# marcottelab/FluorosequencingImageAnalysis

Measured on AMD Instinct MI355X. Metric: psf_lm_fits_per_sec, higher is better.
Workload: dtype f64

## Files before the change

### fluorosequencingimageanalysis_amd/csrc/fsq_fit_rounds.hip

```cpp
#include <algorithm>
#include <atomic>
#include <cstdlib>

#include <mutex>
#include <new>
#include <vector>

#include "fsq_common.h"
#include "fsq_lm_quad.h"

namespace {

#define WAVE_SYNC() do { __builtin_amdgcn_fence(__ATOMIC_RELEASE, "wavefront"); __builtin_amdgcn_wave_barrier(); \
                         __builtin_amdgcn_fence(__ATOMIC_ACQUIRE, "wavefront"); } while (0)

#ifdef FSQ_DEBUG_HZ
__device__ unsigned long long g_hz[32];
#endif
#ifdef FSQ_PHASE_PROFILE
__device__ unsigned long long g_rphase[32];
#define RPH_DECL unsigned long long rph_t0 = clock64(), rph_acc[16] = {0,0,0,0,0,0,0,0,0,0,0,0,0,0,0,0};
#define RPH_MARK(k) { unsigned long long t_ = clock64(); rph_acc[k] += t_ - rph_t0; rph_t0 = t_; }
#define RPH_FLUSH(off) if (threadIdx.x == 0 && (blockIdx.x & 63) == 0) { for (int k_ = 0; k_ < 16; k_++) atomicAdd(&g_rphase[(off) + k_], rph_acc[k_]); }
#else
#define RPH_DECL
#define RPH_MARK(k)
#define RPH_FLUSH(off)
#endif

enum { CNT_A = 0, CNT_BLO = 1, CNT_BHI = 2, CNT_C1 = 3, CNT_C3 = 4, CNT_SET = 8 };
enum { Q_EPS = Q_WA3 };
enum { A_IDX = 0, A_X = 1, A_DIAG = 8, A_LLIM1 = 15, A_FNORM = 16, A_PAR = 17, A_DELTA = 18, A_XNORM = 19, A_ITER = 20,
       A_HDR = 21 , A_E = 21 , A_LEN = 46,
       B_GNORM = 21, B_IPVT = 22, B_QTF = 23, B_SDIAG = 30, B_R = 37, B_LEN = 65,
       C_PARL = 65, C_PARU = 66, C_FP = 67, C_LMIT = 68, C_LEN = 69 };

struct FitOut {
    double x[FSQ_NP];
    int status, niter, nfev, pad;
};
struct FitStat {
    double vmax, vmean;
};

struct Ctx {
    uint16_t* roi;
    int pix32;
    FitOut* out;
    FitStat* stat;
    long long cap;
    long long pool;
    int* err;
    int* slow_total;
    int* done;
    int tshift;
    int wave_prio;
    int force_redo;
    int force_slow_mod;
};

enum { G_KINIT_POS = 1, G_KINIT_SLOT = 2, G_KA_BLO = 3, G_KA_BHI = 4, G_KA_OVERLAP = 5, G_KA_SLOW = 6, G_KB_C1 = 7, G_KB_C3 = 8, G_KB_A = 9,
       G_KB_BLO = 10, G_KB_BHI = 11 };
FSQ_DEV long long fsq_guard(const Ctx& c, long long v, long long limit, int code)
{
    if ((unsigned long long)v < (unsigned long long)limit) return v;
    atomicMax(c.err, code);
    return 0;
}

FSQ_DEV int wave_reserve(int* counter, bool want)
{
    const unsigned long long m = __ballot(want);
    if (m == 0) return 0;
    const int lane = threadIdx.x & 63;
    const int leader = __ffsll((long long)m) - 1;
    int base = 0;
    if (lane == leader) base = atomicAdd(counter, __popcll(m));
    base = __shfl(base, leader);
    return base + __popcll(m & ((1ull << lane) - 1ull));
}

FSQ_DEV long long wave_reserve_checked(const Ctx& c, int* counter, bool want, long long limit, int code)
{
    const int at = wave_reserve(counter, want);
    return want ? fsq_guard(c, at, limit, code) : 0;
}

struct BatchArgs {
    const uint16_t* src; const int32_t* cand; int H, W; long long n; int from_image;
    int pix_fmt;
    long long base;
    int ticket;
    int no_queue;
};

FSQ_DEV void wave_mark_done(int* done, bool term, int ticket)
{
    unsigned long long m = __ballot(term);
    const int lane = threadIdx.x & 63;
    while (m) {
        const int leader = __ffsll((long long)m) - 1;
        const int t = __shfl(ticket, leader);
        const unsigned long long mm = __ballot(term && ticket == t);
        if (lane == leader) atomicAdd(done + t, __popcll(mm));
        m &= ~mm;
    }
}

#ifndef FSQ_NT
#define FSQ_NT 0
#endif
typedef unsigned fsq_u4v __attribute__((ext_vector_type(4)));
FSQ_DEV double nt_ld(const double* p) { return FSQ_NT ? __builtin_nontemporal_load(p) : *p; }
FSQ_DEV void nt_st(double* p, double v) { if (FSQ_NT) __builtin_nontemporal_store(v, p); else *p = v; }
FSQ_DEV uint4 nt_ld4(const void* p)
{
    const fsq_u4v v = FSQ_NT ? __builtin_nontemporal_load((const fsq_u4v*)p) : *(const fsq_u4v*)p;
    return make_uint4(v.x, v.y, v.z, v.w);
}
FSQ_DEV void nt_st4(void* p, uint4 w)
{
    fsq_u4v v; v.x = w.x; v.y = w.y; v.z = w.z; v.w = w.w;
    if (FSQ_NT) __builtin_nontemporal_store(v, (fsq_u4v*)p); else *(fsq_u4v*)p = v;
}
struct NtRef {
    double* p;
    FSQ_DEV operator double() const { return nt_ld(p); }
    FSQ_DEV void operator=(double v) const { nt_st(p, v); }
};
struct NtQ {
    double* p;
    FSQ_DEV NtRef operator[](long long i) const { return NtRef{p + i}; }
};
FSQ_DEV NtQ ntq(const double* p) { return NtQ{const_cast<double*>(p)}; }

FSQ_DEV int tag_slot(const Ctx& c, int tag) { return (int)((unsigned)tag & ((1u << c.tshift) - 1u)); }
FSQ_DEV int tag_ticket(const Ctx& c, int tag) { return (int)((unsigned)tag >> c.tshift); }

FSQ_DEV int rpk(int i, int k) { return i * 7 - (i * (i - 1)) / 2 + (k - i); }
FSQ_DEV double pack2(int a, int b) { return __longlong_as_double(((long long)(unsigned)a) | ((long long)b << 32)); }
FSQ_DEV void unpack2(double v, int* a, int* b) { long long u = __double_as_longlong(v); *a = (int)(unsigned)(u & 0xffffffffll); *b = (int)(u >> 32); }

FSQ_DEV void roi_pixels(const BatchArgs& c, long long idx, double* d)
{
    if (c.from_image) {
        const int f = c.cand[3 * idx], h = c.cand[3 * idx + 1], w = c.cand[3 * idx + 2];
        const size_t base = ((size_t)f * c.H + (h - 2)) * c.W + (w - 2);
#pragma unroll
        for (int a = 0; a < 5; a++)
#pragma unroll
            for (int b = 0; b < 5; b++) d[a * 5 + b] = (double)fsq_pixel(c.src, base + (size_t)a * c.W + b, c.pix_fmt);
    } else {
#pragma unroll
        for (int k = 0; k < FSQ_NPIX; k++) d[k] = (double)c.src[idx * FSQ_NPIX + k];
    }
}

FSQ_DEV void roi_compact(const Ctx& c, long long idx, double* d)
{
    if (c.pix32) {
        const uint32_t* s32 = (const uint32_t*)c.roi + (size_t)idx * 32;
#pragma unroll
        for (int k = 0; k < FSQ_NPIX; k++) d[k] = (double)s32[k];
        return;
    }
    const uint16_t* src = c.roi + (size_t)idx * 32;
    const uint4 a = nt_ld4(src), b = nt_ld4(src + 8), e = nt_ld4(src + 16), f = nt_ld4(src + 24);
    const unsigned w[16] = {a.x, a.y, a.z, a.w, b.x, b.y, b.z, b.w, e.x, e.y, e.z, e.w, f.x, f.y, f.z, f.w};
#pragma unroll
    for (int k = 0; k < FSQ_NPIX; k++) d[k] = (double)((w[k >> 1] >> (16 * (k & 1))) & 0xffffu);
}

__global__ void __launch_bounds__(256) kinit(Ctx c, BatchArgs b, double* __restrict__ QA, int* __restrict__ cntA)
{
    const long long i0 = (long long)blockIdx.x * blockDim.x + threadIdx.x;
    const bool ok = i0 < b.n;
    const long long i = ok ? i0 : 0;
    const long long pos = wave_reserve_checked(c, cntA, ok && !b.no_queue, c.cap, G_KINIT_POS);
    if (b.n <= 0) return;
    const long long slot = fsq_guard(c, b.base + i, c.pool, G_KINIT_SLOT);
    double v[FSQ_NPIX];
    roi_pixels(b, i, v);
    if (ok && c.pix32) {
        uint32_t* dst = (uint32_t*)c.roi + (size_t)slot * 32;
#pragma unroll
        for (int k = 0; k < 32; k++) dst[k] = (k < FSQ_NPIX) ? (unsigned)v[k] : 0u;
    } else if (ok) {
        unsigned w[16];
#pragma unroll
        for (int k = 0; k < 16; k++) {
            unsigned lo = (2 * k < FSQ_NPIX) ? (unsigned)v[2 * k] : 0u, hi = (2 * k + 1 < FSQ_NPIX) ? (unsigned)v[2 * k + 1] : 0u;
            w[k] = lo | (hi << 16);
        }
        uint16_t* dst = c.roi + (size_t)slot * 32;
        nt_st4(dst, make_uint4(w[0], w[1], w[2], w[3])); nt_st4(dst + 8, make_uint4(w[4], w[5], w[6], w[7]));
        nt_st4(dst + 16, make_uint4(w[8], w[9], w[10], w[11])); nt_st4(dst + 24, make_uint4(w[12], w[13], w[14], w[15]));
    }
    double mx = v[0], isum = 0.0;
#pragma unroll
    for (int k = 0; k < FSQ_NPIX; k++) { mx = v[k] > mx ? v[k] : mx; isum += v[k]; }
#pragma unroll
    for (int pass = 0; pass < FSQ_NPIX; pass++)
#pragma unroll
        for (int k = (pass & 1); k + 1 < FSQ_NPIX; k += 2) {
// ... 62 lines not shown
}
template <int G>
FSQ_DEV double kag_dot25(const double* lds, int grp, int off)
{
    double S[4];
#pragma unroll
    for (int l = 0; l < 4; l++) {
        double a = QL(off, l), b = QL(off, 4 + l), c = QL(off, 8 + l), e = QL(off, 12 + l);
        S[l] = ((a * a + b * b) + c * c) + e * e;
    }
    double d = (S[0] + S[2]) + (S[1] + S[3]);
#pragma unroll
    for (int i = 16; i < 25; i++) { double v = QL(off, i); d = fsq_fma(v, v, d); }
    return d;
}

#define KA_ROWS(i) do { if (L == 8 && ((i) % 5) == 4) __builtin_amdgcn_sched_barrier(0); } while (0)
#define KA_PIN(v) do { if (FAST) asm volatile("" : "+v"(v)); } while (0)
#ifdef FSQ_DEBUG_HZ
#define KA_HZ(code, cond) do { if (cond) { hz = true; if (FAST) atomicAdd(&g_hz[code], 1ull); } } while (0)
#else
#define KA_HZ(code, cond) do { if (cond) hz = true; } while (0)
#endif
template <bool FAST, int L, bool P32 = false>
__global__ void __launch_bounds__(64, (L == 8 ? 4 : 2)) kA_jacobian(Ctx c, const double* __restrict__ QA, const int* __restrict__ cntA_p,
                                                                    double* __restrict__ QB, int* __restrict__ cnt_cur,
                                                                    double* __restrict__ SQ, int* __restrict__ slow_cnt,
                                                                    int* __restrict__ next_counters)
{
    constexpr int G = 64 / L;
    constexpr int NC = 8 / L;
    constexpr int MPX = (FSQ_NPIX + L - 1) / L;
    constexpr int MREC = (A_HDR + L - 1) / L;
    __shared__ double lds[Q_KA_END * G];
    const int lane = threadIdx.x, grp = lane / L, cl = lane % L, gbase = lane - cl;
    const int n7 = FSQ_NP;
    if (c.wave_prio) __builtin_amdgcn_s_setprio(3);
    const int cntA = FAST ? *cntA_p : *slow_cnt;
    if (!FAST && blockIdx.x == 0 && threadIdx.x == 0 && cntA > 0) atomicAdd(c.slow_total, cntA);
    if (FAST && blockIdx.x == 0 && threadIdx.x < CNT_SET) next_counters[threadIdx.x] = 0;
    double col[NC][FSQ_NPIX];
    RPH_DECL
    const long long cap = c.cap;
    const int stride = gridDim.x * G;
    int base = blockIdx.x * G;
    if (base >= cntA) return;
    do {
        RPH_MARK(0)
        const bool active = (base + grp) < cntA;
        const NtQ qa = ntq(QA + (active ? base + grp : 0));
        double rec[MREC];
#pragma unroll
        for (int m = 0; m < MREC; m++) { const int f = cl + L * m; rec[m] = (active && f < A_HDR) ? (double)qa[f * cap] : 0.0; }
        bool hz = false, qhz = false;
        int emin = 0;
        int tag, niter, nfev, hist;
        unpack2(__shfl(rec[A_IDX / L], gbase + A_IDX % L), &tag, &hist);
        unpack2(__shfl(rec[A_ITER / L], gbase + A_ITER % L), &niter, &nfev);
        const bool b_hi = hist > 1;
        const int at_lo = wave_reserve(cnt_cur + CNT_BLO, active && cl == 0 && !b_hi);
        const int at_hi = wave_reserve(cnt_cur + CNT_BHI, active && cl == 0 && b_hi);
#ifdef FSQ_EXPERIMENT_EXTRA_ATOMICS_KA
        {
            int sink = 0;
            for (int x = 0; x < FSQ_EXPERIMENT_EXTRA_ATOMICS_KA; x++) sink += wave_reserve(cnt_cur + 5 + (x & 1), active && cl == 0);
            if (sink == 0x7fffffff) atomicMax(c.err, 99);
        }
#endif
        if (active && cl == 0) {
            if (!b_hi) fsq_guard(c, at_lo, cap, G_KA_BLO); else fsq_guard(c, at_hi, cap, G_KA_BHI);
            if ((long long)at_lo + (long long)at_hi + 2 > cap && (at_lo > 0 || at_hi > 0)) {
                const int nlo = b_hi ? cnt_cur[CNT_BLO] : at_lo + 1, nhi = b_hi ? at_hi + 1 : cnt_cur[CNT_BHI];
                if ((long long)nlo + nhi > cap) atomicMax(c.err, (int)G_KA_OVERLAP);
            }
        }
        const long long at = __shfl((active && cl == 0) ? (int)fsq_guard(c, b_hi ? (long long)(cap - 1) - at_hi : (long long)at_lo, cap, b_hi ? G_KA_BHI : G_KA_BLO) : 0, gbase);
        const int idx = tag_slot(c, tag);
        const bool fresh = active && (nfev == 0);
        double llim1 = 0., fnorm = 0., xnorm = 0., delta = 0., par_in = 0.;
        unsigned ipvt = 0x76543210u;
        int status = 0;
        double gnorm = 0.;
        uint4 roi = make_uint4(0u, 0u, 0u, 0u);
        uint4 roi_hi = make_uint4(0u, 0u, 0u, 0u);
        double ev[MPX];
#pragma unroll
        for (int m = 0; m < MPX; m++) ev[m] = 0.0;
        if (active) {
            if (P32) {
                static_assert(!P32 || L == 4, "32-bit pixels: the four-lane Jacobian round only");
                const uint32_t* r32 = (const uint32_t*)c.roi + (size_t)idx * 32 + cl * 8;
                roi = nt_ld4(r32); roi_hi = nt_ld4(r32 + 4);
            } else if (L == 4) roi = nt_ld4(c.roi + (size_t)idx * 32 + cl * 8);
            else {
                const unsigned long long w8 = fsq_bits(nt_ld((const double*)(c.roi + (size_t)idx * 32 + cl * 4)));
                roi.x = (unsigned)w8; roi.y = (unsigned)(w8 >> 32);
            }
            if (!fresh) {
#pragma unroll
                for (int m = 0; m < MPX; m++) { const int k = cl + L * m; if (k < FSQ_NPIX) ev[m] = qa[(A_E + k) * cap]; }
            }
#pragma unroll
            for (int m = 0; m < MREC; m++) {
                const int f = cl + L * m;
                if (f >= 1 && f <= 19) QL(Q_X, f - 1) = rec[m];
            }
        }
        WAVE_SYNC();
        RPH_MARK(1)
        if (active) {
            double xx[FSQ_NP], hh[FSQ_NP];
#pragma unroll
            for (int k = 0; k < FSQ_NP; k++) {
                xx[k] = QL(Q_X, k);
                const double eps = 1.4901161193847656e-08;
                double h_ = eps * __builtin_fabs(xx[k]);
                if (h_ == 0) h_ = eps;
                const double ul = k < 2 ? 0.0 : k < 4 ? 3.0 : k < 6 ? 2.0 : 360.0;
                if (k >= 2 && (xx[k] > ul - h_)) h_ = -h_;
                hh[k] = h_;
            }
            bool bad = false;
            double sn, cs;
            fsq_sincos(FSQ_PI_180 * xx[6], &sn, &cs);
            const double rcx = xx[3] * cs - xx[2] * sn, rcy = xx[3] * sn + xx[2] * cs;
            const FsqDivisor k4 = fsq_divisor(xx[4]), k5 = fsq_divisor(xx[5]);
            if (FAST)
                hz = hz || !fsq_divisor_in_range(xx[4]) || !fsq_divisor_in_range(xx[5]) || !(__builtin_fabs(xx[2]) <= 0x1p100) ||
                     !(__builtin_fabs(xx[3]) <= 0x1p100);
            {
                const unsigned w[4] = {roi.x, roi.y, roi.z, roi.w};
                const unsigned w32[8] = {roi.x, roi.y, roi.z, roi.w, roi_hi.x, roi_hi.y, roi_hi.z, roi_hi.w};
#pragma unroll
                for (int t = 0; t < 32 / L; t++) {
                    const int k = cl * (32 / L) + t;
                    if (k < FSQ_NPIX) QL(Q_DATA, k) = P32 ? (double)w32[t & 7] : (double)((w[t >> 1] >> (16 * (t & 1))) & 0xffffu);
                }
                if (!fresh) {
#pragma unroll
                    for (int m = 0; m < MPX; m++) { const int k = cl + L * m; if (k < FSQ_NPIX) QL(Q_FVEC, k) = ev[m]; }
                }
            }
            WAVE_SYNC();
            if (__ballot(fresh)) {
                if (fresh) {
#pragma unroll 1
                    for (int m = 0; m < MPX; m++) {
                        const int i = cl + L * m;
                        if (i < FSQ_NPIX) {
                            const int xi = i / 5;
                            const double x = (double)xi, y = (double)(i - 5 * xi);
                            const double xp = x * cs - y * sn, yp = x * sn + y * cs;
                            const double E = ka_gauss<FAST>(rcx - xp, rcy - yp, k4, k5, &emin, &bad);
                            QL(Q_FVEC, i) = E;
                        }
                    }
                }
                WAVE_SYNC();
            }
            if (fresh) nfev = 1;
            {
                const double x2p = xx[2] + hh[2], x3p = xx[3] + hh[3];
                const double rcx2 = xx[3] * cs - x2p * sn, rcy2 = xx[3] * sn + x2p * cs;
                const double rcx3 = x3p * cs - xx[2] * sn, rcy3 = x3p * sn + xx[2] * cs;
                if (FAST) KA_HZ(0, !(__builtin_fabs(x2p) <= 0x1p100) || !(__builtin_fabs(x3p) <= 0x1p100));
#pragma unroll 1
                for (int m = 0; m < MPX; m++) {
                    const int i = cl + L * m;
                    if (i < FSQ_NPIX) {
                        const int xi = i / 5;
                        const double x = (double)xi, y = (double)(i - 5 * xi);
                        const double xp = x * cs - y * sn, yp = x * sn + y * cs;
                        const double d = QL(Q_DATA, i);
                        const double E2 = ka_gauss<FAST>(rcx2 - xp, rcy2 - yp, k4, k5, &emin, &bad);
                        const double E3 = ka_gauss<FAST>(rcx3 - xp, rcy3 - yp, k4, k5, &emin, &bad);
                        QL(Q_STAGE, i) = d - (xx[0] + xx[1] * E2);
                        QL(Q_STAGE + 25, i) = d - (xx[0] + xx[1] * E3);
                    }
                }
                const double p0 = (cl == 0) ? xx[0] + hh[0] : xx[0], p1 = (cl == 1) ? xx[1] + hh[1] : xx[1];
#pragma unroll
                for (int i = 0; i < FSQ_NPIX; i++) { col[0][i] = QL(Q_DATA, i) - (p0 + p1 * QL(Q_FVEC, i)); KA_ROWS(i); }
                WAVE_SYNC();
// ... 342 lines not shown
                    col[pass][FSQ_NPIX - 1] = 0.0;
                }
                WAVE_SYNC();
                RPH_MARK(11)
            }
            RPH_MARK(4)
#define QRG(i, k) QL(Q_R, (i) * 7 + nib_get(ipvt, (k)))
            llim1 = QL(Q_TMP, 0); fnorm = QL(Q_TMP, 1); par_in = QL(Q_TMP, 2); delta = QL(Q_TMP, 3); xnorm = QL(Q_TMP, 4);
            if (niter == 1) {
#pragma unroll
                for (int k = 0; k < FSQ_NP; k++) {
                    double a = QL(Q_ACN, k);
                    double dg = (a == 0) ? 1. : a;
                    QL(Q_DIAG, k) = dg;
                    QL(Q_WA3, k) = dg * QL(Q_X, k);
                }
                xnorm = fsq_sqrt(kag_dot7<G>(lds, grp, Q_WA3));
                delta = 100. * xnorm;
                if (delta == 0.) delta = 100.;
            }
            gnorm = 0.;
            if (fnorm != 0) {
                for (int j = 0; j < n7; j++) {
                    double an = QL(Q_ACN, nib_get(ipvt, j));
                    if (an != 0) {
                        double sg = 0.0;
                        for (int i = 0; i <= j; i++) sg += QRG(i, j) * QL(Q_QTF, i);
                        sg = sg / fnorm;
                        gnorm = np_max2(gnorm, __builtin_fabs(sg / an));
                    }
                }
            }
            if (gnorm <= 1e-10) status = 4;
            else {
#pragma unroll
                for (int k = 0; k < FSQ_NP; k++) { double dg = QL(Q_DIAG, k), an = QL(Q_ACN, k); QL(Q_DIAG, k) = (dg > an) ? dg : an; }
            }
            RPH_MARK(5)
            if (FAST) {
                KA_HZ(13, (emin < -FSQ_DIV_EN));
                if (c.force_slow_mod > 0 && (idx % c.force_slow_mod) == 0) hz = true;
                const unsigned long long m = __ballot(hz);
                qhz = ((m >> gbase) & ((1ull << L) - 1ull)) != 0;
            }
            if (status != 0 && cl == 0 && !qhz) {
                FitOut o;
#pragma unroll
                for (int k = 0; k < FSQ_NP; k++) o.x[k] = QL(Q_X, k);
                o.status = status; o.niter = niter; o.nfev = nfev; o.pad = 0;
                c.out[idx] = o;
            }
        }
        wave_mark_done(c.done, active && status != 0 && cl == 0 && !qhz, tag_ticket(c, tag));
        {
            bool go = active && (status == 0);
            if (FAST) {
                int sat = (int)wave_reserve_checked(c, slow_cnt, qhz && cl == 0, cap, G_KA_SLOW);
                sat = __shfl(sat, gbase);
                if (qhz) for (int f = cl; f < A_LEN; f += L) nt_st(SQ + (size_t)sat + f * cap, qa[f * cap]);
                go = go && !qhz;
            }
            const NtQ qb = ntq(QB + at);
            if (go) {
                for (int e = cl; e < 28; e += L) {
                    int i = 0, rem = e;
                    while (rem >= 7 - i) { rem -= 7 - i; i++; }
                    qb[(B_R + e) * cap] = QRG(i, i + rem);
                }
                for (int k = cl; k < FSQ_NP; k += L) {
                    qb[(A_X + k) * cap] = QL(Q_X, k);
                    qb[(A_DIAG + k) * cap] = QL(Q_DIAG, k);
                    qb[(B_QTF + k) * cap] = QL(Q_QTF, k);
                    qb[(B_SDIAG + k) * cap] = 0.;
                }
                if (cl == 0) {
                    qb[A_IDX * cap] = pack2(tag, hist);
                    qb[A_LLIM1 * cap] = llim1; qb[A_FNORM * cap] = fnorm; qb[A_PAR * cap] = par_in; qb[A_DELTA * cap] = delta;
                    qb[A_XNORM * cap] = xnorm; qb[A_ITER * cap] = pack2(niter, nfev);
                    qb[B_GNORM * cap] = gnorm; qb[B_IPVT * cap] = pack2((int)ipvt, 0);
                }
            } else if (active && cl == 0) qb[A_IDX * cap] = pack2(-1, 0);
        }
        RPH_MARK(6)
        base += stride;
    } while (!FAST && base < cntA);
    RPH_FLUSH(16)
}
#undef QRG
#undef REFL
#undef KA_ROWS
#undef KA_PIN
#undef KA_HZ
#pragma pop_macro("QL")

#ifndef FSQ_KA_LANES_DEFAULT
#define FSQ_KA_LANES_DEFAULT 4
#endif
#ifndef FSQ_LMPAR_FIRST
#define FSQ_LMPAR_FIRST 5
#endif
#ifndef FSQ_LMPAR_LO
#define FSQ_LMPAR_LO 1
#endif
#ifndef FSQ_KB_WAVES
#define FSQ_KB_WAVES 2
#endif
FSQ_DEV int kb_res_slot(int i) { return i < 14 ? i : i + 7; }

template <bool FAST>
FSQ_DEV bool kb_trial_gauss(const double* p, double* myscr)
{
    bool bad = false;
    int em = 0;
    double s, c;
    fsq_sincos(FSQ_PI_180 * p[6], &s, &c);
    const double rcen_x = p[3] * c - p[2] * s;
    const double rcen_y = p[3] * s + p[2] * c;
    const FsqDivisor k4 = fsq_divisor(p[4]), k5 = fsq_divisor(p[5]);
    if (FAST)
        bad = !fsq_divisor_in_range(p[4]) || !fsq_divisor_in_range(p[5]) || !(__builtin_fabs(p[2]) <= 0x1p100) ||
              !(__builtin_fabs(p[3]) <= 0x1p100);
#pragma unroll 1
    for (int xi = 0; xi < 5; xi++) {
        const double x = (double)xi;
#pragma unroll
        for (int yi = 0; yi < 5; yi++) {
            const double y = (double)yi;
            const double xp = x * c - y * s;
            const double yp = x * s + y * c;
            const double nu = rcen_x - xp, nv = rcen_y - yp;
            if (FAST) { em = min(em, fsq_expo(nu)); em = min(em, fsq_expo(nv)); }
            const double u = fsq_div_sel<FAST>(nu, k4);
            const double v = fsq_div_sel<FAST>(nv, k5);
            const double e = -(u * u + v * v) / 2.;
            myscr[kb_res_slot(xi * 5 + yi) * 64] = FAST ? fsq_exp_bf(e, &bad) : fsq_exp(e);
        }
    }
    if (FAST) bad = bad || (em < -FSQ_DIV_EN);
    return bad;
}

FSQ_DEV double kb_late_load(const NtRef r) { asm volatile("" ::: "memory"); return (double)r; }

struct KbLimits { int lim[4]; };
template <bool ALIASED, bool P32 = false>
__global__ void __launch_bounds__(64, FSQ_KB_WAVES) kB_step(Ctx c, const double* __restrict__ QB, const double* __restrict__ QC,
                                                  const int* __restrict__ cnt_cur,
                                                  double* __restrict__ QA_next, double* __restrict__ QB_next, double* __restrict__ QC_next,
                                                  int* __restrict__ cnt_next, KbLimits lims)
{
    __shared__ double scr[32 * 64];
    if (c.wave_prio) __builtin_amdgcn_s_setprio(3);
    const int lane = threadIdx.x;
    const long long cap = c.cap;
    double* myscr = scr + lane;
    RPH_DECL
    {
        int b = blockIdx.x, seg, cnt;
        const int n_lo = cnt_cur[CNT_BLO], n_hi = cnt_cur[CNT_BHI], n_c1 = cnt_cur[CNT_C1], n_c3 = cnt_cur[CNT_C3];
        if (b < (n_c3 + 63) / 64) { seg = 3; cnt = n_c3; }
        else if ((b -= (n_c3 + 63) / 64) < (n_hi + 63) / 64) { seg = 1; cnt = n_hi; }
        else if ((b -= (n_hi + 63) / 64) < (n_c1 + 63) / 64) { seg = 2; cnt = n_c1; }
        else if ((b -= (n_c1 + 63) / 64) < (n_lo + 63) / 64) { seg = 0; cnt = n_lo; }
        else return;
        const bool resume = seg >= 2;
        const int lm_limit = lims.lim[seg];
        const int base = b * 64;
        RPH_MARK(0)
        bool live = (base + lane) < cnt;
        const int p_in = live ? (base + lane) : base;
        const NtQ qb = ntq((resume ? QC : QB) + ((seg & 1) ? cap - 1 - p_in : p_in));
        int tag = 0, dummy, niter = 1, nfev = 1, ipvt_i = 0x76543210;
        {
            int t;
            unpack2(qb[A_IDX * cap], &t, &dummy);
            if (t == -1) live = false;
            if (live) tag = t;
        }
        QuadLm q;
        double xq[FSQ_NP];
        double llim1 = 0., fnorm = 1., par = 0., delta = 1., xnorm = 1., fnorm1;
        if (live) {
            unpack2(qb[A_ITER * cap], &niter, &nfev);
            unpack2(qb[B_IPVT * cap], &ipvt_i, &dummy);
#pragma unroll
            for (int i = 0; i < FSQ_NP; i++)
#pragma unroll
                for (int k = 0; k < FSQ_NP; k++) q.r[i][k] = (k >= i) ? (double)qb[(B_R + rpk(i, k)) * cap] : 0.0;
#pragma unroll
            for (int k = 0; k < FSQ_NP; k++) {
                q.qtf[k] = qb[(B_QTF + k) * cap]; q.dg[k] = qb[(A_DIAG + k) * cap]; q.sdiag[k] = qb[(B_SDIAG + k) * cap];
                xq[k] = qb[(A_X + k) * cap];
            }
            llim1 = qb[A_LLIM1 * cap];
            fnorm = qb[A_FNORM * cap]; par = qb[A_PAR * cap]; delta = qb[A_DELTA * cap]; xnorm = qb[A_XNORM * cap];
        } else {
            const double x0[FSQ_NP] = {100., 1000., 2.5, 2.5, 1., 1., 0.};
#pragma unroll
            for (int i = 0; i < FSQ_NP; i++)
#pragma unroll
                for (int k = 0; k < FSQ_NP; k++) q.r[i][k] = (k == i) ? 1.0 : 0.0;
#pragma unroll
            for (int k = 0; k < FSQ_NP; k++) { q.qtf[k] = 0.; q.dg[k] = 1.; q.sdiag[k] = 0.; xq[k] = x0[k]; }
        }
        const unsigned ipvt = (unsigned)ipvt_i;
#define KB_GNORM() kb_late_load(qb[B_GNORM * cap])
#pragma unroll
        for (int k = 0; k < FSQ_NP; k++) myscr[k * 64] = q.dg[k];
#pragma unroll
        for (int j = 0; j < FSQ_NP; j++) q.dgp[j] = myscr[nib_get(ipvt, j) * 64];

        RPH_MARK(1)
        int lm_hist = 0;
        {
            QuadLmparSt st;
            if (!resume) quadlm_lmpar_begin<ALIASED, 64>(q, myscr, ipvt, delta, par, st);
            else if (live) {
                int it, dm;
                unpack2(qb[C_LMIT * cap], &it, &dm);
                st.par = par; st.parl = qb[C_PARL * cap]; st.paru = qb[C_PARU * cap]; st.fp = qb[C_FP * cap];
                st.iter = it; st.done = false;
            } else { st.par = 0.; st.parl = 0.; st.paru = 0.; st.fp = 0.; st.iter = 10; st.done = true; }
            RPH_MARK(7)
            quadlm_lmpar_run<ALIASED, 64>(q, myscr, ipvt, delta, st, lm_limit);
            par = st.par;
            lm_hist = st.iter;
            {
                const bool park = live && !st.done;
                const bool to_c1 = (st.iter < lims.lim[2]);
                const int at1 = (int)wave_reserve_checked(c, cnt_next + CNT_C1, park && to_c1, cap, G_KB_C1);
                const int at3 = (int)wave_reserve_checked(c, cnt_next + CNT_C3, park && !to_c1, cap, G_KB_C3);
                if (park) {
                    const NtQ qn = ntq(QC_next + (to_c1 ? (long long)at1 : cap - 1 - at3));
                    qn[A_IDX * cap] = pack2(tag, 0);
#pragma unroll
                    for (int k = 0; k < FSQ_NP; k++) {
                        qn[(A_X + k) * cap] = xq[k]; qn[(A_DIAG + k) * cap] = q.dg[k];
                        qn[(B_QTF + k) * cap] = q.qtf[k]; qn[(B_SDIAG + k) * cap] = q.sdiag[k];
                    }
                    qn[A_LLIM1 * cap] = llim1; qn[A_FNORM * cap] = fnorm; qn[A_PAR * cap] = par; qn[A_DELTA * cap] = delta;
                    qn[A_XNORM * cap] = xnorm; qn[A_ITER * cap] = pack2(niter, nfev);
                    qn[B_GNORM * cap] = KB_GNORM(); qn[B_IPVT * cap] = pack2((int)ipvt, 0);
#pragma unroll
                    for (int i = 0; i < FSQ_NP; i++)
#pragma unroll
                        for (int k = i; k < FSQ_NP; k++) qn[(B_R + rpk(i, k)) * cap] = q.r[i][k];
                    qn[C_PARL * cap] = st.parl; qn[C_PARU * cap] = st.paru; qn[C_FP * cap] = st.fp;
                    qn[C_LMIT * cap] = pack2(st.iter, 0);
                }
                live = live && !park;
            }
        }
        RPH_MARK(2)
        double wa1[FSQ_NP], wa2[FSQ_NP];
        bool lpeg[FSQ_NP], upeg[FSQ_NP];
        int nlpeg = 0, nupeg = 0;
#pragma unroll
        for (int k = 0; k < FSQ_NP; k++) {
            wa1[k] = -q.xp[k];
            lpeg[k] = (xq[k] == fsq_llim(k, llim1)); nlpeg += lpeg[k];
            upeg[k] = fsq_qulim(k) && (xq[k] == fsq_ulim(k)); nupeg += upeg[k];
        }
        double alpha = 1.;
        if (nlpeg > 0) {
            double mxw = wa1[0];
#pragma unroll
            for (int k = 1; k < FSQ_NP; k++) mxw = np_max2(mxw, wa1[k]);
#pragma unroll
            for (int k = 0; k < FSQ_NP; k++) if (lpeg[k]) wa1[k] = np_clip(wa1[k], 0., mxw);
        }
        if (nupeg > 0) {
            double mnw = wa1[0];
#pragma unroll
            for (int k = 1; k < FSQ_NP; k++) mnw = np_min2(mnw, wa1[k]);
#pragma unroll
            for (int k = 0; k < FSQ_NP; k++) if (upeg[k]) wa1[k] = np_clip(wa1[k], mnw, 0.);
        }
        {
            bool any = false; double tmin = 0.;
#pragma unroll
            for (int k = 0; k < FSQ_NP; k++)
                if ((__builtin_fabs(wa1[k]) > FSQ_MACHEP) && ((xq[k] + wa1[k]) < fsq_llim(k, llim1))) {
                    double t = (fsq_llim(k, llim1) - xq[k]) / wa1[k];
                    tmin = any ? np_min2(tmin, t) : t; any = true;
                }
            if (any) alpha = np_min2(alpha, tmin);
            any = false;
#pragma unroll
            for (int k = 0; k < FSQ_NP; k++)
                if ((__builtin_fabs(wa1[k]) > FSQ_MACHEP) && fsq_qulim(k) && ((xq[k] + wa1[k]) > fsq_ulim(k))) {
                    double t = (fsq_ulim(k) - xq[k]) / wa1[k];
                    tmin = any ? np_min2(tmin, t) : t; any = true;
                }
            if (any) alpha = np_min2(alpha, tmin);
        }
        double pnorm = 0.0;
#pragma unroll
        for (int k = 0; k < FSQ_NP; k++) {
            wa1[k] = wa1[k] * alpha;
            wa2[k] = xq[k] + wa1[k];
            const double ul = fsq_ulim(k), ll = fsq_llim(k, llim1);
            double sgnu = (ul >= 0) * 2. - 1., sgnl = (ll >= 0) * 2. - 1.;
            double ulim1 = ul * (1 - sgnu * FSQ_MACHEP) - (ul == 0) * FSQ_MACHEP;
            double llim1_ = ll * (1 + sgnl * FSQ_MACHEP) + (ll == 0) * FSQ_MACHEP;
            if (fsq_qulim(k) && (wa2[k] >= ulim1)) wa2[k] = ul;
            if (wa2[k] <= llim1_) wa2[k] = ll;
            double t = q.dg[k] * wa1[k];
            pnorm = fsq_fma(t, t, pnorm);
            myscr[(14 + k) * 64] = wa1[k];
        }
        pnorm = fsq_sqrt(pnorm);
        if (niter == 1) delta = np_min2(delta, pnorm);
        RPH_MARK(3)
        {
            asm volatile("" ::: "memory");
            bool redo = kb_trial_gauss<true>(wa2, myscr);
#ifdef FSQ_EXPERIMENT_TRIAL_TWICE
            asm volatile("" ::: "memory");
            redo = kb_trial_gauss<true>(wa2, myscr) || redo;
            asm volatile("" ::: "memory");
#endif
            if (c.force_slow_mod > 0 && (tag_slot(c, tag) % c.force_slow_mod) == 0) redo = true;
            if (__ballot(redo)) {
                if (redo) kb_trial_gauss<false>(wa2, myscr);
            }
            const uint16_t* src = c.roi + (size_t)tag_slot(c, tag) * 32;
            unsigned w[P32 ? 28 : 16];
            if (P32) {
                const uint32_t* s32 = (const uint32_t*)c.roi + (size_t)tag_slot(c, tag) * 32;
#pragma unroll
                for (int g = 0; g < 7; g++) { const uint4 q4 = nt_ld4(s32 + 4 * g); w[4 * g] = q4.x; w[4 * g + 1] = q4.y; w[4 * g + 2] = q4.z; w[4 * g + 3] = q4.w; }
            } else {
                const uint4 a = nt_ld4(src), b = nt_ld4(src + 8), e = nt_ld4(src + 16), f = nt_ld4(src + 24);
                const unsigned w16[16] = {a.x, a.y, a.z, a.w, b.x, b.y, b.z, b.w, e.x, e.y, e.z, e.w, f.x, f.y, f.z, f.w};
#pragma unroll
                for (int g = 0; g < 16; g++) w[g] = w16[g];
            }
            double S[4], d = 0.0;
#pragma unroll
            for (int i = 0; i < FSQ_NPIX; i++) {
                const double pix = P32 ? (double)w[i] : (double)((w[i >> 1] >> (16 * (i & 1))) & 0xffffu);
                const double r = pix - (wa2[0] + wa2[1] * myscr[kb_res_slot(i) * 64]);
                if (i < 4) S[i] = r * r;
                else if (i < 16) S[i & 3] = S[i & 3] + r * r;
                else {
                    if (i == 16) d = (S[0] + S[2]) + (S[1] + S[3]);
                    d = fsq_fma(r, r, d);
                }
            }
            fnorm1 = fsq_sqrt(d);
        }
        nfev++;
        RPH_MARK(4)
        double actred = -1.;
        if ((0.1 * fnorm1) < fnorm) actred = -fsq_pow2(fnorm1 / fnorm) + 1.;
        double wa3[FSQ_NP];
#pragma unroll
        for (int k = 0; k < FSQ_NP; k++) wa3[k] = 0.;
#pragma unroll
        for (int j = 0; j < FSQ_NP; j++) {
            wa3[j] = 0;
            double wj = myscr[(14 + nib_get(ipvt, j)) * 64];
#pragma unroll
            for (int i = 0; i < FSQ_NP; i++)
                if (i <= j) wa3[i] = wa3[i] + q.r[i][j] * wj;
        }
        double t1s = 0.0;
#pragma unroll
        for (int k = 0; k < FSQ_NP; k++) { double t = alpha * wa3[k]; t1s = fsq_fma(t, t, t1s); }
        double temp1 = fsq_sqrt(t1s) / fnorm;
        double temp2 = (fsq_sqrt(alpha * par) * pnorm) / fnorm;
        double prered = temp1 * temp1 + (temp2 * temp2) / 0.5;
        double dirder = -(temp1 * temp1 + temp2 * temp2);
        double ratio = 0.;
        if (prered != 0) ratio = actred / prered;
        if (ratio <= 0.25) {
            double temp;
            if (actred >= 0) temp = .5;
            else temp = .5 * dirder / (dirder + .5 * actred);
            if (((0.1 * fnorm1) >= fnorm) || (temp < 0.1)) temp = 0.1;
            delta = temp * np_min2(delta, pnorm / 0.1);
            par = par / temp;
        } else if ((par == 0) || (ratio >= 0.75)) {
            delta = pnorm / .5;
            par = .5 * par;
        }
        const bool accepted = (ratio >= 0.0001);
        if (accepted) {
            double xs = 0.0;
#pragma unroll
            for (int k = 0; k < FSQ_NP; k++) {
                xq[k] = wa2[k];
                double t = q.dg[k] * wa2[k];
                xs = fsq_fma(t, t, xs);
            }
            xnorm = fsq_sqrt(xs);
            fnorm = fnorm1;
            niter = niter + 1;
        }
        int status = 0;
        bool c1 = (__builtin_fabs(actred) <= 1e-10) && (prered <= 1e-10) && (0.5 * ratio <= 1);
        if (c1) status = 1;
        if (delta <= 1e-10 * xnorm) status = 2;
        if (c1 && (status == 2)) status = 3;
        if (status == 0) {
            if (niter >= 200) status = 5;
            if ((__builtin_fabs(actred) <= FSQ_MACHEP) && (prered <= FSQ_MACHEP) && (0.5 * ratio <= 1)) status = 6;
            if (delta <= FSQ_MACHEP * xnorm) status = 7;
            if (KB_GNORM() <= FSQ_MACHEP) status = 8;
        }
        if (status == 0 && !accepted) {
            bool fin = __builtin_isfinite(ratio);
#pragma unroll
            for (int k = 0; k < FSQ_NP; k++)
                fin = fin && __builtin_isfinite(wa1[k]) && __builtin_isfinite(wa2[k]) && __builtin_isfinite(xq[k]);
            if (!fin) status = -16;
        }
        RPH_MARK(5)
        if (live && status != 0) {
            FitOut o;
#pragma unroll
            for (int k = 0; k < FSQ_NP; k++) o.x[k] = xq[k];
            o.status = status; o.niter = niter; o.nfev = nfev; o.pad = 0;
            c.out[tag_slot(c, tag)] = o;
        }
        wave_mark_done(c.done, live && status != 0, tag_ticket(c, tag));
        {
            const bool toA = live && status == 0 && accepted, toB = live && status == 0 && !accepted;
            const bool hi = lm_hist > 1;
#ifdef FSQ_EXPERIMENT_EXTRA_ATOMICS_KB
            {
                int sink = 0;
                for (int x = 0; x < FSQ_EXPERIMENT_EXTRA_ATOMICS_KB; x++) sink += wave_reserve(cnt_next + 5 + (x & 1), live);
                if (sink == 0x7fffffff) atomicMax(c.err, 99);
            }
#endif
            const int atA = (int)wave_reserve_checked(c, cnt_next + CNT_A, toA, cap, G_KB_A);
            const int atBl = (int)wave_reserve_checked(c, cnt_next + CNT_BLO, toB && !hi, cap, G_KB_BLO);
            const int atBh = (int)wave_reserve_checked(c, cnt_next + CNT_BHI, toB && hi, cap, G_KB_BHI);
            if (toA || toB) {
                const NtQ qn = ntq(toA ? (QA_next + atA) : (QB_next + (hi ? cap - 1 - atBh : (long long)atBl)));
                qn[A_IDX * cap] = pack2(tag, lm_hist);
#pragma unroll
                for (int k = 0; k < FSQ_NP; k++) { qn[(A_X + k) * cap] = xq[k]; qn[(A_DIAG + k) * cap] = q.dg[k]; }
                qn[A_LLIM1 * cap] = llim1; qn[A_FNORM * cap] = fnorm; qn[A_PAR * cap] = par; qn[A_DELTA * cap] = delta;
                qn[A_XNORM * cap] = xnorm; qn[A_ITER * cap] = pack2(niter, nfev);
                if (toA) {
#pragma unroll
                    for (int i = 0; i < FSQ_NPIX; i++) qn[(A_E + i) * cap] = myscr[kb_res_slot(i) * 64];
                }
                if (toB) {
                    qn[B_GNORM * cap] = KB_GNORM(); qn[B_IPVT * cap] = pack2((int)ipvt, 0);
#pragma unroll
                    for (int k = 0; k < FSQ_NP; k++) { qn[(B_QTF + k) * cap] = q.qtf[k]; qn[(B_SDIAG + k) * cap] = q.sdiag[k]; }
#undef KB_GNORM
#pragma unroll
                    for (int i = 0; i < FSQ_NP; i++)
#pragma unroll
                        for (int k = i; k < FSQ_NP; k++) qn[(B_R + rpk(i, k)) * cap] = q.r[i][k];
                }
            }
        }
        RPH_MARK(6)
    }
    RPH_FLUSH(0)
}

__global__ void __launch_bounds__(64) kfinish(Ctx c, BatchArgs b, FsqRow* __restrict__ rows)
{
    long long i = (long long)blockIdx.x * blockDim.x + threadIdx.x;
    if (i >= b.n) return;
    const long long slot = b.base + i;
    const FitOut S = c.out[slot];
    double data[FSQ_NPIX], p[FSQ_NP];
    roi_compact(c, slot, data);
#pragma unroll
    for (int k = 0; k < FSQ_NP; k++) p[k] = S.x[k];
    const double vmax = c.stat[slot].vmax, vmean = c.stat[slot].vmean;
    int h = 2, w = 2, field = 0;
    if (b.from_image) { field = b.cand[3 * i]; h = b.cand[3 * i + 1]; w = b.cand[3 * i + 2]; }
    double fit[FSQ_NPIX];
    fsq_model(p, fit);
    double num = 0.0, den = 0.0, rm = 0.0;
    for (int k = 0; k < FSQ_NPIX; k++) { double d = data[k] - fit[k]; num += d * d; }
    for (int k = 0; k < FSQ_NPIX; k++) { double d = data[k] - vmean; den += d * d; }
    for (int k = 0; k < FSQ_NPIX; k++) rm += fsq_pow2(data[k] - fit[k]);
    FsqRow r;
    r.h0 = p[2] + h - 2.5;
    r.w0 = p[3] + w - 2.5;
    r.H = p[0]; r.A = p[1]; r.sigma_h = p[4]; r.sigma_w = p[5]; r.theta = p[6];
    r.rmse = fsq_sqrt(rm / 25.0);
    r.r2 = 1.0 - num / den;
    {
        double op[16];
        int t = 0;
        for (int ww = 0; ww < 5; ww++) op[t++] = data[ww];
        for (int ww = 0; ww < 5; ww++) op[t++] = data[20 + ww];
        for (int hh = 1; hh < 4; hh++) { op[t++] = data[hh * 5]; op[t++] = data[hh * 5 + 4]; }
        double isum = 0.0;
        for (int k = 0; k < 16; k++) isum += op[k];
        double mean = isum / 16.0, rr[8];
        for (int k = 0; k < 8; k++) { double d0 = op[k] - mean, d1 = op[8 + k] - mean; rr[k] = d0 * d0 + d1 * d1; }
        double res = ((rr[0] + rr[1]) + (rr[2] + rr[3])) + ((rr[4] + rr[5]) + (rr[6] + rr[7]));
        res = 0.0 + res;
        r.s_n = (vmax - mean) / fsq_sqrt(res / 16.0);
    }
    r.p2 = p[2]; r.p3 = p[3];
    r.h = h; r.w = w; r.field = field;
// ... 521 lines not shown
```

Before: 21.42 million.

## Split wave atomics into issue/finish and hoist global loads earlier in LM kernels

Splits the wave-level atomic reservation into an issue half and a finish half, so the kA counter atomics are issued early and their results consumed only after the fit work, hiding atomic latency. It hoists the residual and ROI pixel loads and the gnorm and C-stage state loads to the start of the kernels, caching gnorm in shared scratch instead of re-reading global memory late. It also specialises the image ROI gather per pixel format and removes some compiler memory barriers. In exchange it raises register and LDS pressure, and it now loads ev even for fresh fits.

```diff
diff --git a/fluorosequencingimageanalysis_amd/csrc/fsq_fit_rounds.hip b/fluorosequencingimageanalysis_amd/csrc/fsq_fit_rounds.hip
--- a/fluorosequencingimageanalysis_amd/csrc/fsq_fit_rounds.hip
+++ b/fluorosequencingimageanalysis_amd/csrc/fsq_fit_rounds.hip
@@ -68,22 +68,41 @@
     return 0;
 }
 
-FSQ_DEV int wave_reserve(int* counter, bool want)
-{
-    const unsigned long long m = __ballot(want);
-    if (m == 0) return 0;
+struct WaveRes {
+    unsigned long long m;
+    int raw;
+};
+FSQ_DEV WaveRes wave_reserve_issue(int* counter, bool want)
+{
+    WaveRes r;
+    r.m = __ballot(want);
+    r.raw = 0;
+    if (r.m == 0) return r;
     const int lane = threadIdx.x & 63;
-    const int leader = __ffsll((long long)m) - 1;
-    int base = 0;
-    if (lane == leader) base = atomicAdd(counter, __popcll(m));
-    base = __shfl(base, leader);
-    return base + __popcll(m & ((1ull << lane) - 1ull));
-}
-
+    const int leader = __ffsll((long long)r.m) - 1;
+    int off = 0;
+    asm volatile("" : "+v"(off));
+    if (lane == leader) r.raw = atomicAdd(counter + off, __popcll(r.m));
+    return r;
+}
+FSQ_DEV int wave_reserve_finish(const WaveRes& r)
+{
+    if (r.m == 0) return 0;
+    const int lane = threadIdx.x & 63;
+    const int leader = __ffsll((long long)r.m) - 1;
+    const int base = __shfl(r.raw, leader);
+    return base + __popcll(r.m & ((1ull << lane) - 1ull));
+}
+FSQ_DEV int wave_reserve(int* counter, bool want) { return wave_reserve_finish(wave_reserve_issue(counter, want)); }
+
+FSQ_DEV long long wave_reserve_finish_checked(const Ctx& c, const WaveRes& r, bool want, long long limit, int code)
+{
+    const int at = wave_reserve_finish(r);
+    return want ? fsq_guard(c, at, limit, code) : 0;
+}
 FSQ_DEV long long wave_reserve_checked(const Ctx& c, int* counter, bool want, long long limit, int code)
 {
-    const int at = wave_reserve(counter, want);
-    return want ? fsq_guard(c, at, limit, code) : 0;
+    return wave_reserve_finish_checked(c, wave_reserve_issue(counter, want), want, limit, code);
 }
 
 struct BatchArgs {
@@ -146,10 +165,12 @@
     if (c.from_image) {
         const int f = c.cand[3 * idx], h = c.cand[3 * idx + 1], w = c.cand[3 * idx + 2];
         const size_t base = ((size_t)f * c.H + (h - 2)) * c.W + (w - 2);
-#pragma unroll
-        for (int a = 0; a < 5; a++)
-#pragma unroll
-            for (int b = 0; b < 5; b++) d[a * 5 + b] = (double)fsq_pixel(c.src, base + (size_t)a * c.W + b, c.pix_fmt);
+#define ROI_ROWS(fmt) _Pragma("unroll") for (int a = 0; a < 5; a++) _Pragma("unroll") for (int b = 0; b < 5; b++) \
+                          d[a * 5 + b] = (double)fsq_pixel(c.src, base + (size_t)a * c.W + b, (fmt))
+        if (c.pix_fmt == FSQ_PIXELS_U16) { ROI_ROWS(FSQ_PIXELS_U16); }
+        else if (c.pix_fmt == FSQ_PIXELS_U32) { ROI_ROWS(FSQ_PIXELS_U32); }
+        else { ROI_ROWS(FSQ_PIXELS_F16); }
+#undef ROI_ROWS
     } else {
 #pragma unroll
         for (int k = 0; k < FSQ_NPIX; k++) d[k] = (double)c.src[idx * FSQ_NPIX + k];
@@ -318,29 +339,15 @@
         double rec[MREC];
 #pragma unroll
         for (int m = 0; m < MREC; m++) { const int f = cl + L * m; rec[m] = (active && f < A_HDR) ? (double)qa[f * cap] : 0.0; }
+        double ev[MPX];
+#pragma unroll
+        for (int m = 0; m < MPX; m++) { const int k = cl + L * m; ev[m] = (active && k < FSQ_NPIX) ? (double)qa[(A_E + k) * cap] : 0.0; }
         bool hz = false, qhz = false;
         int emin = 0;
         int tag, niter, nfev, hist;
         unpack2(__shfl(rec[A_IDX / L], gbase + A_IDX % L), &tag, &hist);
         unpack2(__shfl(rec[A_ITER / L], gbase + A_ITER % L), &niter, &nfev);
         const bool b_hi = hist > 1;
-        const int at_lo = wave_reserve(cnt_cur + CNT_BLO, active && cl == 0 && !b_hi);
-        const int at_hi = wave_reserve(cnt_cur + CNT_BHI, active && cl == 0 && b_hi);
-#ifdef FSQ_EXPERIMENT_EXTRA_ATOMICS_KA
-        {
-            int sink = 0;
-            for (int x = 0; x < FSQ_EXPERIMENT_EXTRA_ATOMICS_KA; x++) sink += wave_reserve(cnt_cur + 5 + (x & 1), active && cl == 0);
-            if (sink == 0x7fffffff) atomicMax(c.err, 99);
-        }
-#endif
-        if (active && cl == 0) {
-            if (!b_hi) fsq_guard(c, at_lo, cap, G_KA_BLO); else fsq_guard(c, at_hi, cap, G_KA_BHI);
-            if ((long long)at_lo + (long long)at_hi + 2 > cap && (at_lo > 0 || at_hi > 0)) {
-                const int nlo = b_hi ? cnt_cur[CNT_BLO] : at_lo + 1, nhi = b_hi ? at_hi + 1 : cnt_cur[CNT_BHI];
-                if ((long long)nlo + nhi > cap) atomicMax(c.err, (int)G_KA_OVERLAP);
-            }
-        }
-        const long long at = __shfl((active && cl == 0) ? (int)fsq_guard(c, b_hi ? (long long)(cap - 1) - at_hi : (long long)at_lo, cap, b_hi ? G_KA_BHI : G_KA_BLO) : 0, gbase);
         const int idx = tag_slot(c, tag);
         const bool fresh = active && (nfev == 0);
         double llim1 = 0., fnorm = 0., xnorm = 0., delta = 0., par_in = 0.;
@@ -349,9 +356,6 @@
         double gnorm = 0.;
         uint4 roi = make_uint4(0u, 0u, 0u, 0u);
         uint4 roi_hi = make_uint4(0u, 0u, 0u, 0u);
-        double ev[MPX];
-#pragma unroll
-        for (int m = 0; m < MPX; m++) ev[m] = 0.0;
         if (active) {
             if (P32) {
                 static_assert(!P32 || L == 4, "32-bit pixels: the four-lane Jacobian round only");
@@ -362,10 +366,17 @@
                 const unsigned long long w8 = fsq_bits(nt_ld((const double*)(c.roi + (size_t)idx * 32 + cl * 4)));
                 roi.x = (unsigned)w8; roi.y = (unsigned)(w8 >> 32);
             }
-            if (!fresh) {
-#pragma unroll
-                for (int m = 0; m < MPX; m++) { const int k = cl + L * m; if (k < FSQ_NPIX) ev[m] = qa[(A_E + k) * cap]; }
-            }
+        }
+        const WaveRes res_lo = wave_reserve_issue(cnt_cur + CNT_BLO, active && cl == 0 && !b_hi);
+        const WaveRes res_hi = wave_reserve_issue(cnt_cur + CNT_BHI, active && cl == 0 && b_hi);
+#ifdef FSQ_EXPERIMENT_EXTRA_ATOMICS_KA
+        {
+            int sink = 0;
+            for (int x = 0; x < FSQ_EXPERIMENT_EXTRA_ATOMICS_KA; x++) sink += wave_reserve(cnt_cur + 5 + (x & 1), active && cl == 0);
+            if (sink == 0x7fffffff) atomicMax(c.err, 99);
+        }
+#endif
+        if (active) {
 #pragma unroll
             for (int m = 0; m < MREC; m++) {
                 const int f = cl + L * m;
@@ -395,6 +406,7 @@
                 hz = hz || !fsq_divisor_in_range(xx[4]) || !fsq_divisor_in_range(xx[5]) || !(__builtin_fabs(xx[2]) <= 0x1p100) ||
                      !(__builtin_fabs(xx[3]) <= 0x1p100);
             {
+                asm volatile("" :: "v"(rcx), "v"(rcy) : "memory");
                 const unsigned w[4] = {roi.x, roi.y, roi.z, roi.w};
                 const unsigned w32[8] = {roi.x, roi.y, roi.z, roi.w, roi_hi.x, roi_hi.y, roi_hi.z, roi_hi.w};
 #pragma unroll
@@ -843,6 +855,18 @@
             }
         }
         wave_mark_done(c.done, active && status != 0 && cl == 0 && !qhz, tag_ticket(c, tag));
+        long long at;
+        {
+            const int at_lo = wave_reserve_finish(res_lo), at_hi = wave_reserve_finish(res_hi);
+            if (active && cl == 0) {
+                if (!b_hi) fsq_guard(c, at_lo, cap, G_KA_BLO); else fsq_guard(c, at_hi, cap, G_KA_BHI);
+                if ((long long)at_lo + (long long)at_hi + 2 > cap && (at_lo > 0 || at_hi > 0)) {
+                    const int nlo = b_hi ? cnt_cur[CNT_BLO] : at_lo + 1, nhi = b_hi ? at_hi + 1 : cnt_cur[CNT_BHI];
+                    if ((long long)nlo + nhi > cap) atomicMax(c.err, (int)G_KA_OVERLAP);
+                }
+            }
+            at = __shfl((active && cl == 0) ? (int)fsq_guard(c, b_hi ? (long long)(cap - 1) - at_hi : (long long)at_lo, cap, b_hi ? G_KA_BHI : G_KA_BLO) : 0, gbase);
+        }
         {
             bool go = active && (status == 0);
             if (FAST) {
@@ -931,8 +955,7 @@
     return bad;
 }
 
-FSQ_DEV double kb_late_load(const NtRef r) { asm volatile("" ::: "memory"); return (double)r; }
-
+enum { KB_GNORM_SLOT = 32, KB_SCR = 33 };
 struct KbLimits { int lim[4]; };
 template <bool ALIASED, bool P32 = false>
 __global__ void __launch_bounds__(64, FSQ_KB_WAVES) kB_step(Ctx c, const double* __restrict__ QB, const double* __restrict__ QC,
@@ -940,7 +963,7 @@
                                                   double* __restrict__ QA_next, double* __restrict__ QB_next, double* __restrict__ QC_next,
                                                   int* __restrict__ cnt_next, KbLimits lims)
 {
-    __shared__ double scr[32 * 64];
+    __shared__ double scr[KB_SCR * 64];
     if (c.wave_prio) __builtin_amdgcn_s_setprio(3);
     const int lane = threadIdx.x;
     const long long cap = c.cap;
@@ -971,6 +994,7 @@
         QuadLm q;
         double xq[FSQ_NP];
         double llim1 = 0., fnorm = 1., par = 0., delta = 1., xnorm = 1., fnorm1;
+        double c_parl = 0., c_paru = 0., c_fp = 0., c_lmit = 0.;
         if (live) {
             unpack2(qb[A_ITER * cap], &niter, &nfev);
             unpack2(qb[B_IPVT * cap], &ipvt_i, &dummy);
@@ -985,7 +1009,10 @@
             }
             llim1 = qb[A_LLIM1 * cap];
             fnorm = qb[A_FNORM * cap]; par = qb[A_PAR * cap]; delta = qb[A_DELTA * cap]; xnorm = qb[A_XNORM * cap];
+            myscr[KB_GNORM_SLOT * 64] = qb[B_GNORM * cap];
+            if (resume) { c_parl = qb[C_PARL * cap]; c_paru = qb[C_PARU * cap]; c_fp = qb[C_FP * cap]; c_lmit = qb[C_LMIT * cap]; }
         } else {
+            myscr[KB_GNORM_SLOT * 64] = 1.;
             const double x0[FSQ_NP] = {100., 1000., 2.5, 2.5, 1., 1., 0.};
 #pragma unroll
             for (int i = 0; i < FSQ_NP; i++)
@@ -995,7 +1022,6 @@
             for (int k = 0; k < FSQ_NP; k++) { q.qtf[k] = 0.; q.dg[k] = 1.; q.sdiag[k] = 0.; xq[k] = x0[k]; }
         }
         const unsigned ipvt = (unsigned)ipvt_i;
-#define KB_GNORM() kb_late_load(qb[B_GNORM * cap])
 #pragma unroll
         for (int k = 0; k < FSQ_NP; k++) myscr[k * 64] = q.dg[k];
 #pragma unroll
@@ -1003,13 +1029,14 @@
 
         RPH_MARK(1)
         int lm_hist = 0;
+        unsigned w[P32 ? 28 : 16];
         {
             QuadLmparSt st;
             if (!resume) quadlm_lmpar_begin<ALIASED, 64>(q, myscr, ipvt, delta, par, st);
             else if (live) {
                 int it, dm;
-                unpack2(qb[C_LMIT * cap], &it, &dm);
-                st.par = par; st.parl = qb[C_PARL * cap]; st.paru = qb[C_PARU * cap]; st.fp = qb[C_FP * cap];
+                unpack2(c_lmit, &it, &dm);
+                st.par = par; st.parl = c_parl; st.paru = c_paru; st.fp = c_fp;
                 st.iter = it; st.done = false;
             } else { st.par = 0.; st.parl = 0.; st.paru = 0.; st.fp = 0.; st.iter = 10; st.done = true; }
             RPH_MARK(7)
@@ -1017,10 +1044,25 @@
             par = st.par;
             lm_hist = st.iter;
             {
+                if (P32) {
+                    const uint32_t* s32 = (const uint32_t*)c.roi + (size_t)tag_slot(c, tag) * 32;
+#pragma unroll
+                    for (int g = 0; g < 7; g++) { const uint4 q4 = nt_ld4(s32 + 4 * g); w[4 * g] = q4.x; w[4 * g + 1] = q4.y; w[4 * g + 2] = q4.z; w[4 * g + 3] = q4.w; }
+                } else {
+                    const uint16_t* src = c.roi + (size_t)tag_slot(c, tag) * 32;
+                    const uint4 a = nt_ld4(src), b = nt_ld4(src + 8), e = nt_ld4(src + 16), f = nt_ld4(src + 24);
+                    const unsigned w16[16] = {a.x, a.y, a.z, a.w, b.x, b.y, b.z, b.w, e.x, e.y, e.z, e.w, f.x, f.y, f.z, f.w};
+#pragma unroll
+                    for (int g = 0; g < 16; g++) w[g] = w16[g];
+                }
+            }
+            {
                 const bool park = live && !st.done;
                 const bool to_c1 = (st.iter < lims.lim[2]);
-                const int at1 = (int)wave_reserve_checked(c, cnt_next + CNT_C1, park && to_c1, cap, G_KB_C1);
-                const int at3 = (int)wave_reserve_checked(c, cnt_next + CNT_C3, park && !to_c1, cap, G_KB_C3);
+                const WaveRes res1 = wave_reserve_issue(cnt_next + CNT_C1, park && to_c1);
+                const WaveRes res3 = wave_reserve_issue(cnt_next + CNT_C3, park && !to_c1);
+                const int at1 = (int)wave_reserve_finish_checked(c, res1, park && to_c1, cap, G_KB_C1);
+                const int at3 = (int)wave_reserve_finish_checked(c, res3, park && !to_c1, cap, G_KB_C3);
                 if (park) {
                     const NtQ qn = ntq(QC_next + (to_c1 ? (long long)at1 : cap - 1 - at3));
                     qn[A_IDX * cap] = pack2(tag, 0);
@@ -1031,7 +1073,7 @@
                     }
                     qn[A_LLIM1 * cap] = llim1; qn[A_FNORM * cap] = fnorm; qn[A_PAR * cap] = par; qn[A_DELTA * cap] = delta;
                     qn[A_XNORM * cap] = xnorm; qn[A_ITER * cap] = pack2(niter, nfev);
-                    qn[B_GNORM * cap] = KB_GNORM(); qn[B_IPVT * cap] = pack2((int)ipvt, 0);
+                    qn[B_GNORM * cap] = myscr[KB_GNORM_SLOT * 64]; qn[B_IPVT * cap] = pack2((int)ipvt, 0);
 #pragma unroll
                     for (int i = 0; i < FSQ_NP; i++)
 #pragma unroll
@@ -1104,7 +1146,6 @@
         if (niter == 1) delta = np_min2(delta, pnorm);
         RPH_MARK(3)
         {
-            asm volatile("" ::: "memory");
             bool redo = kb_trial_gauss<true>(wa2, myscr);
 #ifdef FSQ_EXPERIMENT_TRIAL_TWICE
             asm volatile("" ::: "memory");
@@ -1114,18 +1155,6 @@
             if (c.force_slow_mod > 0 && (tag_slot(c, tag) % c.force_slow_mod) == 0) redo = true;
             if (__ballot(redo)) {
                 if (redo) kb_trial_gauss<false>(wa2, myscr);
-            }
-            const uint16_t* src = c.roi + (size_t)tag_slot(c, tag) * 32;
-            unsigned w[P32 ? 28 : 16];
-            if (P32) {
-                const uint32_t* s32 = (const uint32_t*)c.roi + (size_t)tag_slot(c, tag) * 32;
-#pragma unroll
-                for (int g = 0; g < 7; g++) { const uint4 q4 = nt_ld4(s32 + 4 * g); w[4 * g] = q4.x; w[4 * g + 1] = q4.y; w[4 * g + 2] = q4.z; w[4 * g + 3] = q4.w; }
-            } else {
-                const uint4 a = nt_ld4(src), b = nt_ld4(src + 8), e = nt_ld4(src + 16), f = nt_ld4(src + 24);
-                const unsigned w16[16] = {a.x, a.y, a.z, a.w, b.x, b.y, b.z, b.w, e.x, e.y, e.z, e.w, f.x, f.y, f.z, f.w};
-#pragma unroll
-                for (int g = 0; g < 16; g++) w[g] = w16[g];
             }
             double S[4], d = 0.0;
 #pragma unroll
@@ -1198,7 +1227,7 @@
             if (niter >= 200) status = 5;
             if ((__builtin_fabs(actred) <= FSQ_MACHEP) && (prered <= FSQ_MACHEP) && (0.5 * ratio <= 1)) status = 6;
             if (delta <= FSQ_MACHEP * xnorm) status = 7;
-            if (KB_GNORM() <= FSQ_MACHEP) status = 8;
+            if (myscr[KB_GNORM_SLOT * 64] <= FSQ_MACHEP) status = 8;
         }
         if (status == 0 && !accepted) {
             bool fin = __builtin_isfinite(ratio);
@@ -1226,9 +1255,12 @@
                 if (sink == 0x7fffffff) atomicMax(c.err, 99);
             }
 #endif
-            const int atA = (int)wave_reserve_checked(c, cnt_next + CNT_A, toA, cap, G_KB_A);
-            const int atBl = (int)wave_reserve_checked(c, cnt_next + CNT_BLO, toB && !hi, cap, G_KB_BLO);
-            const int atBh = (int)wave_reserve_checked(c, cnt_next + CNT_BHI, toB && hi, cap, G_KB_BHI);
+            const WaveRes resA = wave_reserve_issue(cnt_next + CNT_A, toA);
+            const WaveRes resBl = wave_reserve_issue(cnt_next + CNT_BLO, toB && !hi);
+            const WaveRes resBh = wave_reserve_issue(cnt_next + CNT_BHI, toB && hi);
+            const int atA = (int)wave_reserve_finish_checked(c, resA, toA, cap, G_KB_A);
+            const int atBl = (int)wave_reserve_finish_checked(c, resBl, toB && !hi, cap, G_KB_BLO);
+            const int atBh = (int)wave_reserve_finish_checked(c, resBh, toB && hi, cap, G_KB_BHI);
             if (toA || toB) {
                 const NtQ qn = ntq(toA ? (QA_next + atA) : (QB_next + (hi ? cap - 1 - atBh : (long long)atBl)));
                 qn[A_IDX * cap] = pack2(tag, lm_hist);
@@ -1241,10 +1273,9 @@
                     for (int i = 0; i < FSQ_NPIX; i++) qn[(A_E + i) * cap] = myscr[kb_res_slot(i) * 64];
                 }
                 if (toB) {
-                    qn[B_GNORM * cap] = KB_GNORM(); qn[B_IPVT * cap] = pack2((int)ipvt, 0);
+                    qn[B_GNORM * cap] = myscr[KB_GNORM_SLOT * 64]; qn[B_IPVT * cap] = pack2((int)ipvt, 0);
 #pragma unroll
                     for (int k = 0; k < FSQ_NP; k++) { qn[(B_QTF + k) * cap] = q.qtf[k]; qn[(B_SDIAG + k) * cap] = q.sdiag[k]; }
-#undef KB_GNORM
 #pragma unroll
                     for (int i = 0; i < FSQ_NP; i++)
 #pragma unroll
```

Measured after the change: 21.40 million. No clear change (-0.1%).
